# thanh-nt25/Whisper-context-biasing

Hardware: AMD Instinct MI355X
Metric: audio-seconds/sec (RTF) + biased-WER, whisper-small 30s clips, batch32 (higher is better)
Workload: dtype bf16

## Files before the change

whisper_context_biasing_amd/csrc/gemm_impl.h:

```cpp
#pragma once
#include <stdexcept>
#include <string>
#include "common.h"
#include "kernels.h"

#include <algorithm>
#include <cstdio>
#include <cstdlib>
#include <type_traits>

namespace wcb {

WCB_DEV void glds16(const void* gptr, void* lds_wave_base) {
  __builtin_amdgcn_global_load_lds(gptr, (__attribute__((address_space(3))) void*)lds_wave_base, 16, 0, 0);
}

WCB_DEV long a_row(const GemmArgs& g, int m) {
  return g.a_Mb ? (long)(m / g.a_Mb) * g.a_strideB + (long)(m % g.a_Mb) * g.lda : (long)m * g.lda;
}
WCB_DEV long c_row(const GemmArgs& g, int m) {
  return g.c_Mb ? (long)(m / g.c_Mb) * g.c_strideB + (long)(m % g.c_Mb) * g.ldc : (long)m * g.ldc;
}

enum : int { E_BIAS = 1, E_GELU = 2, E_RESID = 4, E_F32 = 8, E_ADDROW = 16, E_HEAD = 32, E_RUNTIME = 1 << 30 };
// ... 181 lines not shown
      for (int i = 0; i < FM; ++i)
#pragma unroll
        for (int j = 0; j < FN; ++j) acc[i][j] = mma16(a[i], b[j], acc[i][j]);
    }
    asm volatile("s_waitcnt vmcnt(0)" ::: "memory");
    __syncthreads();
  }

  constexpr int LDC = BN + 4;
  float* ct = reinterpret_cast<float*>(smem);
#pragma unroll
  for (int j = 0; j < FN; ++j) {
    const int col = wn * TN + j * 16 + (lane & 15);
    const int n = min(n0 + col, g.N - 1);
#pragma unroll
    for (int i = 0; i < FM; ++i)
#pragma unroll
      for (int e = 0; e < 4; ++e) {
        const int row = wm * TM + i * 16 + (lane >> 4) * 4 + e;
        const int m = min(m0 + row, g.M - 1);
        ct[row * LDC + col] = epi_pointwise<T, EPI>(g, m, n, acc[i][j][e]);
      }
  }
  __syncthreads();
  constexpr int C8 = BN / 8;
#pragma unroll 2
  for (int idx = tid; idx < BM * C8; idx += NT) {
    const int row = idx / C8, c8 = idx % C8;
    const int m = m0 + row;
    const int n = n0 + c8 * 8;
    if (m >= g.M || n >= g.N) continue;
    float v[8];
    const f32x4 lo = *reinterpret_cast<const f32x4*>(ct + row * LDC + c8 * 8);
    const f32x4 hi = *reinterpret_cast<const f32x4*>(ct + row * LDC + c8 * 8 + 4);
#pragma unroll
    for (int e = 0; e < 4; ++e) { v[e] = lo[e]; v[e + 4] = hi[e]; }
    epi_store8<T, EPI>(g, m, n, v);
  }
}

template <typename T, int BM, int BN, int WM, int WN, int NS, int EPI, bool LNF = false, int KT = 1, int BKB = 128,
          int PRIO = 0, bool WFM = false>
__global__ __launch_bounds__(WM * WN * 64) void gemm_ring_kernel(GemmArgs g) {
  constexpr int NW = WM * WN, NT = NW * 64;
  static_assert(BKB == 128 || BKB == 64, "LDS row: 128 or 64 bytes");
  constexpr int BK = BKB / 2, CE = 8;
  constexpr int CPR = BKB / 16, RPI = 64 / CPR, KS = BKB / 64;
  constexpr int TM = BM / WM, TN = BN / WN, FM = TM / 16, FN = TN / 16;
  constexpr int SUB = (BM + BN) * BKB, STAGE = SUB * KT;
  constexpr int IA = BM / RPI / NW, IB = BN / RPI / NW, GL = (IA + IB) * KT;
  static_assert(IA * NW * RPI == BM && IB * NW * RPI == BN, "tile rows must split over waves");
  auto swz = [](int r) { return BKB == 128 ? (r >> 1) & 7 : (r >> 2) & 3; };
  using Frag = typename DT<T>::frag;
  extern __shared__ __attribute__((aligned(16))) char smem[];

  const int tid = threadIdx.x, lane = tid & 63, wave = tid >> 6;
  const int wm = wave / WN, wn = wave % WN;
  const int tiles_n = (g.N + BN - 1) / BN;
  const int wg = xcd_remap(blockIdx.x, gridDim.x);
  int m0, n0;
  if (g.raster > 0) {
    const int tiles_m = (g.M + BM - 1) / BM, band = g.raster * tiles_n;
    const int fm = (wg / band) * g.raster, gm = min(tiles_m - fm, g.raster), r = wg % band;
    m0 = (fm + r % gm) * BM;
    n0 = (r / gm) * BN;
  } else {
    m0 = (wg / tiles_n) * BM;
    n0 = (wg % tiles_n) * BN;
  }

  const T* A = reinterpret_cast<const T*>(g.A);
  const T* W = reinterpret_cast<const T*>(g.W);
  const T* a_src[IA];
  const T* b_src[IB];
#pragma unroll
  for (int i = 0; i < IA; ++i) {
    const int r = (wave + i * NW) * RPI + lane / CPR;
    const int m = min(m0 + r, g.M - 1);
    a_src[i] = A + a_row(g, m) + ((lane % CPR) ^ swz(r)) * CE;
  }
  static_assert(!WFM || BKB == 128, "fragment-major W: 64-deep sub-tiles");
#pragma unroll
  for (int i = 0; i < IB; ++i) {
    const int r = (wave + i * NW) * RPI + lane / CPR;
    const long n = min(n0 + r, g.N - 1);
    const int c = (lane % CPR) ^ swz(r);
    if constexpr (WFM)
      b_src[i] = reinterpret_cast<const T*>(g.W_fm) + ((n / 16) * (g.K / 32) + c / 4) * 512 + (16 * (c % 4) + n % 16) * 8;
    else
      b_src[i] = W + n * g.ldw + c * CE;
  }
  constexpr int WKS = WFM ? 16 : 1;
  auto stage = [&](int st, int k0) {
#pragma unroll
    for (int t = 0; t < KT; ++t) {
      char* base = smem + st * STAGE + t * SUB;
#pragma unroll
      for (int i = 0; i < IA; ++i) glds16(a_src[i] + k0 + t * BK, base + (wave + i * NW) * 1024);
#pragma unroll
      for (int i = 0; i < IB; ++i) glds16(b_src[i] + (long)(k0 + t * BK) * WKS, base + BM * BKB + (wave + i * NW) * 1024);
    }
  };

  f32x4 acc[FM][FN];
#pragma unroll
  for (int i = 0; i < FM; ++i)
#pragma unroll
    for (int j = 0; j < FN; ++j) acc[i][j] = f32x4{0.f, 0.f, 0.f, 0.f};

  constexpr int LNF_OFF = NS * STAGE > BM * (BN + 4) * 4 ? NS * STAGE : BM * (BN + 4) * 4;
  float* lnraw = reinterpret_cast<float*>(smem + LNF_OFF);
  float* lnst = lnraw + BM * (kLnfMaxK / 32) * 2;
  const int nk = g.K / (BK * KT);
#pragma unroll
  for (int p = 0; p < NS - 1; ++p)
    if (p < nk) stage(p, p * BK * KT);
  if constexpr (LNF) {
    const int per_row = g.rst_nb * 8 / 16;
    const int chunks = BM * per_row;
    for (int q0 = wave * 64; q0 < chunks; q0 += NT) {
      const int q = min(q0 + lane, chunks - 1), r = q / per_row, j = q % per_row;
      const int m = min(m0 + r, g.M - 1);
      glds16(g.rst_in + ((long)m * g.rst_nb) * 2 + j * 4, reinterpret_cast<char*>(lnraw) + (long)q0 * 16);
    }
  }
  int st = 0;
  for (int kt = 0; kt < nk; ++kt) {
    const int ahead = min(nk - 1 - kt, NS - 2);
    if constexpr (NS >= 4) {
      static_assert(4 * GL <= 63, "vmcnt range");
      if (NS >= 6 && ahead >= 4) asm volatile("s_waitcnt vmcnt(%0)" :: "n"(4 * GL) : "memory");
      else if (NS >= 5 && ahead == 3) asm volatile("s_waitcnt vmcnt(%0)" :: "n"(3 * GL) : "memory");
      else if (ahead >= 2) asm volatile("s_waitcnt vmcnt(%0)" :: "n"(2 * GL) : "memory");
      else if (ahead == 1) asm volatile("s_waitcnt vmcnt(%0)" :: "n"(GL) : "memory");
      else asm volatile("s_waitcnt vmcnt(0)" ::: "memory");
    } else if constexpr (NS == 3) {
      if (ahead >= 1) asm volatile("s_waitcnt vmcnt(%0)" :: "n"(GL) : "memory");
      else asm volatile("s_waitcnt vmcnt(0)" ::: "memory");
    } else {
      asm volatile("s_waitcnt vmcnt(0)" ::: "memory");
    }
    __builtin_amdgcn_s_barrier();
    {
      const int nxt = kt + NS - 1;
      int sn = st + NS - 1;
      if (sn >= NS) sn -= NS;
      if (nxt < nk) stage(sn, nxt * BK * KT);
    }
#pragma unroll
    for (int kq = 0; kq < KS * KT; ++kq) {
      const char* base = smem + st * STAGE + (kq / KS) * SUB;
      const int ks = kq % KS;
      Frag a[FM], b[FN];
      const int c = ks * 4 + (lane >> 4);
#pragma unroll
      for (int i = 0; i < FM; ++i) {
        const int r = wm * TM + i * 16 + (lane & 15);
        a[i] = *reinterpret_cast<const Frag*>(base + r * BKB + ((c ^ swz(r)) << 4));
      }
#pragma unroll
      for (int j = 0; j < FN; ++j) {
        const int r = wn * TN + j * 16 + (lane & 15);
        b[j] = *reinterpret_cast<const Frag*>(base + BM * BKB + r * BKB + ((c ^ swz(r)) << 4));
      }
      if constexpr (PRIO == 1) __builtin_amdgcn_s_setprio(1);
#pragma unroll
      for (int i = 0; i < FM; ++i)
#pragma unroll
        for (int j = 0; j < FN; ++j) acc[i][j] = mma16(a[i], b[j], acc[i][j]);
      if constexpr (PRIO == 1) __builtin_amdgcn_s_setprio(0);
    }
    st = st + 1 == NS ? 0 : st + 1;
  }
  if constexpr (LNF) {
    __syncthreads();
    constexpr int LPR = NT / BM;
    static_assert(LPR >= 1 && (LPR & (LPR - 1)) == 0 && LPR <= 64, "lanes per row");
    const int r = tid / LPR, sub = tid % LPR;
    float a1 = 0.f, a2 = 0.f;
    for (int j = sub; j < g.rst_nb; j += LPR) {
      const float2 t = *reinterpret_cast<const float2*>(lnraw + ((long)r * g.rst_nb + j) * 2);
      a1 += t.x;
      a2 += t.y;
    }
#pragma unroll
    for (int o = 1; o < LPR; o <<= 1) { a1 += __shfl_xor(a1, o, 64); a2 += __shfl_xor(a2, o, 64); }
    if (sub == 0) {
      const float mean = a1 / g.K;
      lnst[2 * r] = mean;
      lnst[2 * r + 1] = rsqrtf(fmaxf(a2 / g.K - mean * mean, 0.f) + 1e-5f);
    }
  }
  __syncthreads();

  constexpr int LDC = BN + 4;
  constexpr int PASSES = (BM * LDC * 4 <= 160 * 1024) ? 1 : WM;
  constexpr int PR = BM / PASSES;
  float* ct = reinterpret_cast<float*>(smem);
#pragma unroll
  for (int ps = 0; ps < PASSES; ++ps) {
    if (PASSES == 1 || wm == ps) {
#pragma unroll
      for (int j = 0; j < FN; ++j) {
        const int col = wn * TN + j * 16 + (lane & 15);
#pragma unroll
        for (int i = 0; i < FM; ++i)
#pragma unroll
          for (int e = 0; e < 4; ++e) {
            const int row = wm * TM + i * 16 + (lane >> 4) * 4 + e;
            float v = acc[i][j][e];
            if constexpr (LNF) v = lnst[2 * row + 1] * (v - lnst[2 * row] * g.ln_u[min(n0 + col, g.N - 1)]);
            ct[(row - ps * PR) * LDC + col] = v;
          }
      }
    }
    __syncthreads();
    constexpr int C8 = BN / 8, RPIT = NT / C8;
    const int c8 = tid % C8;
    float b8[8] = {0.f, 0.f, 0.f, 0.f, 0.f, 0.f, 0.f, 0.f};
    if (has<EPI>(g, E_BIAS)) {
      const int nb = min(n0 + c8 * 8, g.N - 8);
      const f32x4 lo = *reinterpret_cast<const f32x4*>(g.bias + nb);
      const f32x4 hi = *reinterpret_cast<const f32x4*>(g.bias + nb + 4);
#pragma unroll
      for (int e = 0; e < 4; ++e) { b8[e] = lo[e]; b8[e + 4] = hi[e]; }
    }
    const int row0 = tid < RPIT * C8 ? tid / C8 : PR;
    constexpr int UNR = PR >= 2 * RPIT && EPI != E_RUNTIME ? 2 : 1;
#pragma unroll UNR
    for (int row = row0; row < PR; row += RPIT) {
      const int m = m0 + ps * PR + row;
      const int n = n0 + c8 * 8;
      const bool ok = m < g.M && n < g.N;
      float v[8];
      const f32x4 lo = *reinterpret_cast<const f32x4*>(ct + row * LDC + c8 * 8);
      const f32x4 hi = *reinterpret_cast<const f32x4*>(ct + row * LDC + c8 * 8 + 4);
#pragma unroll
      for (int e = 0; e < 4; ++e) { v[e] = lo[e]; v[e + 4] = hi[e]; }
#pragma unroll
      for (int e = 0; e < 8; ++e) {
        if (has<EPI>(g, E_BIAS)) v[e] += b8[e];
        if (has<EPI>(g, E_GELU)) v[e] = gelu_t<T>(v[e]);
        if (has<EPI>(g, E_ADDROW))
          v[e] += g.addrow[(long)(g.c_Mb ? min(m, g.M - 1) % g.c_Mb : min(m, g.M - 1)) * g.N + min(n + e, g.N - 1)];
      }
      if (ok) epi_store8<T, EPI>(g, m, n, v);
      if (EPI == E_RUNTIME && g.rst_out) {
        float a1 = 0.f, a2 = 0.f;
#pragma unroll
        for (int e = 0; e < 8; ++e) { a1 += v[e]; a2 = fmaf(v[e], v[e], a2); }
        a1 += __shfl_xor(a1, 1, 64); a2 += __shfl_xor(a2, 1, 64);
        a1 += __shfl_xor(a1, 2, 64); a2 += __shfl_xor(a2, 2, 64);
        if (ok && (c8 & 3) == 0) *reinterpret_cast<float2*>(g.rst_out + ((long)m * (g.N / 32) + n / 32) * 2) = float2{a1, a2};
      }
    }
    if (PASSES > 1) __syncthreads();
  }
}

template <typename T, int BM, int BN, int WM, int WN, int NS, int EPI, bool LNF = false, int KT = 1, int BKB = 128,
          int PRIO = 0, bool WFM = false>
static void launch_ring_e(const GemmArgs& g, hipStream_t s) {
  const int tiles = ((g.M + BM - 1) / BM) * ((g.N + BN - 1) / BN);
  constexpr int ring_bytes = NS * (BM + BN) * BKB * KT;
  constexpr int epi_full = BM * (BN + 4) * 4;
  constexpr int epi_bytes = epi_full <= 160 * 1024 ? epi_full : epi_full / WM;
  constexpr int base = ring_bytes > epi_bytes ? ring_bytes : epi_bytes;
  constexpr int lds = base + (LNF ? BM * (kLnfMaxK / 32) * 2 * 4 + 2 * BM * 4 : 0);
  static_assert(lds <= 160 * 1024, "LDS budget");
  static bool attr_set = false;
  if (!attr_set) {
    (void)hipFuncSetAttribute((const void*)gemm_ring_kernel<T, BM, BN, WM, WN, NS, EPI, LNF, KT, BKB, PRIO, WFM>,
                              hipFuncAttributeMaxDynamicSharedMemorySize, lds);
    attr_set = true;
  }
  WCB_LAUNCH((gemm_ring_kernel<T, BM, BN, WM, WN, NS, EPI, LNF, KT, BKB, PRIO, WFM>), dim3(tiles), dim3(WM * WN * 64), lds, s, g);
}

template <typename T, int BM, int BN, int NS, bool LNF, int KT = 1>
static void launch_ring_dec(const GemmArgs& g, hipStream_t s) {
  if (g.W_fm && g.K % 32 == 0) launch_ring_e<T, BM, BN, 2, 2, NS, E_RUNTIME, LNF, KT, 128, 0, true>(g, s);
  else launch_ring_e<T, BM, BN, 2, 2, NS, E_RUNTIME, LNF, KT>(g, s);
}

template <typename T, int BM, int BN, int WM, int WN, int NS, int BKB = 128, int PRIO = 1>
static void launch_ring(const GemmArgs& g, hipStream_t s) {
  const int bits = (g.bias ? E_BIAS : 0) | (g.act == 1 ? E_GELU : 0) | (g.resid ? E_RESID : 0) |
                   (g.out_f32 ? E_F32 : 0) | (g.addrow ? E_ADDROW : 0) | (g.mode == 1 ? E_HEAD : 0);
  switch (bits) {
    case E_BIAS: launch_ring_e<T, BM, BN, WM, WN, NS, E_BIAS, false, 1, BKB, PRIO>(g, s); break;
    case E_BIAS | E_GELU: launch_ring_e<T, BM, BN, WM, WN, NS, E_BIAS | E_GELU, false, 1, BKB, PRIO>(g, s); break;
    case E_BIAS | E_RESID | E_F32: launch_ring_e<T, BM, BN, WM, WN, NS, E_BIAS | E_RESID | E_F32, false, 1, BKB, PRIO>(g, s); break;
    case E_BIAS | E_GELU | E_F32 | E_ADDROW:
      launch_ring_e<T, BM, BN, WM, WN, NS, E_BIAS | E_GELU | E_F32 | E_ADDROW, false, 1, BKB, PRIO>(g, s); break;
    case E_BIAS | E_HEAD: launch_ring_e<T, BM, BN, WM, WN, NS, E_BIAS | E_HEAD, false, 1, BKB, PRIO>(g, s); break;
    default: launch_ring_e<T, BM, BN, WM, WN, NS, E_RUNTIME, false, 1, BKB, PRIO>(g, s); break;
  }
}

#ifdef WCB_GEMM_PROBE
__device__ unsigned long long* wcb_gemm_probe;
#define GPROBE(k)                                                                              \
  do {                                                                                         \
    if (threadIdx.x == 0) wcb_gemm_probe[blockIdx.x * 8 + (k)] = __builtin_amdgcn_s_memtime(); \
  } while (0)
#else
#define GPROBE(k) do {} while (0)
#endif
__device__ float wcb_pp_zeros[8192];
__device__ __attribute__((aligned(16))) char wcb_pp_scratch[64 * 16];

template <int N> WCB_DEV void vm_wait() { asm volatile("s_waitcnt vmcnt(%0)" :: "n"(N < 63 ? N : 63) : "memory"); }

template <typename T, int EPI, int BN = 256>
__global__ __launch_bounds__(512) void gemm_pp_kernel(GemmArgs g) {
  using Frag = typename DT<T>::frag;
  constexpr int BUF = 65536, WOFF = 32768;
  static_assert(BN == 256 || BN == 192, "tile width");
  constexpr int FW = BN / 64;
  constexpr int OPK = FW + 4;
  constexpr int S = 8 * FW + ((EPI & E_RESID) ? 8 * FW : 0);
  constexpr int BIAS_LDS = 2 * BUF;
  extern __shared__ __attribute__((aligned(16))) char smem[];
  const int tid = threadIdx.x, lane = tid & 63, wave = __builtin_amdgcn_readfirstlane(tid >> 6);
  const int wr = wave >> 2, wc = wave & 3;
  GPROBE(0);
  const int tiles_n = g.N / BN, tiles_m = (g.M + 255) >> 8, ntiles = tiles_m * tiles_n;
  const int nk = g.K >> 6;
  const int my = (ntiles - 1 - (int)blockIdx.x) / (int)gridDim.x + 1;
  const int total = my * nk;
  auto origin = [&](int it, int& m0, int& n0) {
    const int wg = xcd_remap((int)blockIdx.x + it * (int)gridDim.x, ntiles);
    if (g.raster > 0) {
      const int band = g.raster * tiles_n;
      const int fm = (wg / band) * g.raster, gm = min(tiles_m - fm, g.raster), r = wg % band;
      m0 = (fm + r % gm) * 256;
      n0 = (r / gm) * BN;
    } else {
      m0 = (wg / tiles_n) * 256;
      n0 = (wg % tiles_n) * BN;
    }
  };
  auto swzr = [](int r) { return (r >> 1) & 7; };
  const T* A = reinterpret_cast<const T*>(g.A);
  const T* W = reinterpret_cast<const T*>(g.W);
  const int i8 = 8 * wave + (lane >> 3), ch = lane & 7;
  const int m_last = (tiles_m - 1) * 256;
  int aoff[4], aoff_last[4], boff[4];
#pragma unroll
  for (int p = 0; p < 4; ++p) {
    const int ar = i8 < 32 ? 32 * p + i8 : 96 + 32 * p + i8;
    const int cs = (ch ^ swzr(ar)) << 3;
    aoff[p] = ar * (int)g.lda + cs;
    aoff_last[p] = (min(m_last + ar, g.M - 1) - m_last) * (int)g.lda + cs;
    boff[p] = (64 * min(p, FW - 1) + i8) * (int)g.ldw + ((ch ^ swzr(64 * p + i8)) << 3);
  }
  struct Cur { int it, kt, m0, n0; const T* a; const T* b; bool last; };
  auto set_tile = [&](Cur& c) {
    origin(c.it, c.m0, c.n0);
    c.a = A + (long)c.m0 * g.lda;
    c.b = W + (long)c.n0 * g.ldw;
    c.last = c.m0 == m_last;
  };
  auto advance = [&](Cur& c) {
    c.a += 64;
    c.b += 64;
    if (++c.kt == nk) {
      c.kt = 0;
      if (++c.it < my) set_tile(c);
    }
  };
  auto dma_a = [&](int p, const Cur& c, int gk) {
    glds16(c.a + (c.last ? aoff_last[p] : aoff[p]),
           smem + (gk & 1) * BUF + (wave < 4 ? 32 * p + 8 * wave : 96 + 32 * p + 8 * wave) * 128);
  };
  auto dma_b = [&](int t, const Cur& c, int gk) {
    glds16(c.b + boff[t], smem + (gk & 1) * BUF + WOFF + (64 * t + 8 * wave) * 128);
  };
  auto barrier = [] {
    __builtin_amdgcn_sched_barrier(0);
    __builtin_amdgcn_s_barrier();
    __builtin_amdgcn_sched_barrier(0);
  };

  f32x4 acc[8][FW];
#pragma unroll
  for (int i = 0; i < 8; ++i)
#pragma unroll
    for (int j = 0; j < FW; ++j) acc[i][j] = f32x4{0.f, 0.f, 0.f, 0.f};

  Cur cc;
  cc.it = 0; cc.kt = 0;
  set_tile(cc);
  Cur c1 = cc, c2 = cc;
  advance(c1);
  advance(c2);
  advance(c2);
  dma_b(0, cc, 0); dma_b(1, cc, 0); dma_a(0, cc, 0); dma_b(2, cc, 0);
  if constexpr (FW == 4) dma_b(3, cc, 0);
  dma_a(1, cc, 0); dma_a(2, cc, 0); dma_a(3, cc, 0);
  if (total > 1) {
    dma_b(0, c1, 1); dma_b(1, c1, 1); dma_a(0, c1, 1); dma_b(2, c1, 1);
    if constexpr (FW == 4) dma_b(3, c1, 1);
    dma_a(1, c1, 1);
  }
  GPROBE(1);
  if (total > 1) vm_wait<3 + FW + 2>();
  else vm_wait<3>();
  GPROBE(2);
  barrier();
  if (wr == 1) barrier();

  const int c0 = lane >> 4;
  const float* bias = g.bias ? g.bias : wcb_pp_zeros;
  const int sl = (lane >> 1) & 7;
  const int lo0 = (lane & 15) * 128 + ((c0 ^ sl) << 4), lo1 = (lane & 15) * 128 + (((4 + c0) ^ sl) << 4);
  const int wb0 = WOFF + 16 * FW * wc * 128 + lo0, wb1 = WOFF + 16 * FW * wc * 128 + lo1;
  const int ab0 = 128 * wr * 128 + lo0, ab1 = 128 * wr * 128 + lo1;
  auto ktile = [&](int gk, auto steady_tag) {
    constexpr bool ST = decltype(steady_tag)::value;
    const char* buf = smem + (gk & 1) * BUF;
    const bool n1 = ST || gk + 1 < total, n2 = ST || gk + 2 < total;
    const bool e0 = !ST && cc.kt == 0 && cc.it > 0, e1 = !ST && cc.kt == 1 && cc.it > 0;
    const bool plain = ST || (n2 && !e0 && !e1);
    Frag bw[FW][2];
#pragma unroll
    for (int p = 0; p < 4; ++p) {
      if (plain) {
        if (p < 3) vm_wait<OPK>();
        else vm_wait<6>();
      } else if (p == 0) {
        if (n1) { if (e0 || e1) vm_wait<OPK + S>(); else vm_wait<OPK>(); }
        else { if (e0 || e1) vm_wait<2 + S>(); else vm_wait<2>(); }
      } else if (p == 1) {
        if (n1) { if (e0) vm_wait<OPK + S>(); else vm_wait<OPK>(); }
        else { if (e0) vm_wait<1 + S>(); else vm_wait<1>(); }
      } else if (p == 2) {
        if (n1) { if (e0) vm_wait<OPK + S>(); else vm_wait<OPK>(); }
        else { if (e0) vm_wait<S>(); else vm_wait<0>(); }
      } else if (n1) {
        if (n2) { if (e0) vm_wait<6 + S>(); else vm_wait<6>(); }
        else { if (e0) vm_wait<3 + S>(); else vm_wait<3>(); }
      }
      if (p == 0) {
#pragma unroll
        for (int j = 0; j < FW; ++j) {
          bw[j][0] = *reinterpret_cast<const Frag*>(buf + wb0 + j * 16 * 128);
          bw[j][1] = *reinterpret_cast<const Frag*>(buf + wb1 + j * 16 * 128);
        }
      }
      if (!ST && p == 0 && cc.kt == 0 && wave == 0)
        glds16(bias + (BN == 256 ? cc.n0 + 4 * lane : min(cc.n0 + 4 * lane, g.N - 4)), smem + BIAS_LDS + (cc.it & 1) * 1024);
      Frag af[2][2];
#pragma unroll
      for (int i = 0; i < 2; ++i) {
        af[i][0] = *reinterpret_cast<const Frag*>(buf + ab0 + (32 * p + 16 * i) * 128);
        af[i][1] = *reinterpret_cast<const Frag*>(buf + ab1 + (32 * p + 16 * i) * 128);
      }
      if (p == 0 && n1) dma_a(2, c1, gk + 1);
      if (p == 1 && n1) dma_a(3, c1, gk + 1);
      if (p == 2 && n2) { dma_b(0, c2, gk + 2); dma_b(1, c2, gk + 2); dma_a(0, c2, gk + 2); }
      if (p == 3 && n2) {
        dma_b(2, c2, gk + 2);
        if constexpr (FW == 4) dma_b(3, c2, gk + 2);
        dma_a(1, c2, gk + 2);
      }
      barrier();
      asm volatile("s_waitcnt lgkmcnt(0)" ::: "memory");
      __builtin_amdgcn_s_setprio(1);
#pragma unroll
      for (int ks = 0; ks < 2; ++ks)
#pragma unroll
        for (int i = 0; i < 2; ++i)
#pragma unroll
          for (int j = 0; j < FW; ++j) acc[2 * p + i][j] = mma16(bw[j][ks], af[i][ks], acc[2 * p + i][j]);
      __builtin_amdgcn_s_setprio(0);
      barrier();
    }
  };
  for (int gk = 0; gk < total; ++gk) {
    ktile(gk, std::false_type{});
    if (gk == 0) GPROBE(3);
    if (gk == nk / 2) GPROBE(4);
    if (gk == 2 * nk - 1) GPROBE(7);
    if (cc.kt == nk - 1) {
      if (cc.it == 0) GPROBE(5);
      const int rb = cc.m0 + 128 * wr + (lane & 15);
      const int cb = cc.n0 + 16 * FW * wc + 4 * c0;
      f32x4 b4[FW];
#pragma unroll
      for (int j = 0; j < FW; ++j)
        b4[j] = *reinterpret_cast<const f32x4*>(smem + BIAS_LDS + (cc.it & 1) * 1024 + (16 * FW * wc + 4 * c0 + 16 * j) * 4);
#pragma unroll
      for (int mi = 0; mi < 8; ++mi) {
        const int m = rb + 16 * mi;
        const long off = (long)min(m, g.M - 1) * g.ldc + cb;
        f32x4 r4[FW];
        if constexpr ((EPI & E_RESID) != 0) {
#pragma unroll
          for (int j = 0; j < FW; ++j) r4[j] = *reinterpret_cast<const f32x4*>(g.resid + off + 16 * j);
        }
#pragma unroll
        for (int j = 0; j < FW; ++j) {
          f32x4 v = acc[mi][j] + b4[j];
          acc[mi][j] = f32x4{0.f, 0.f, 0.f, 0.f};
          if constexpr ((EPI & E_GELU) != 0) {
#pragma unroll
            for (int e = 0; e < 4; ++e) v[e] = gelu_t<T>(v[e]);
          }
          if constexpr ((EPI & E_RESID) != 0) v += r4[j];
          if constexpr ((EPI & E_F32) != 0) {
            float* dst = m < g.M ? reinterpret_cast<float*>(g.out) + off + 16 * j
                                 : reinterpret_cast<float*>(wcb_pp_scratch + lane * 16);
            *reinterpret_cast<f32x4*>(dst) = v;
          } else {
            typedef short s4 __attribute__((ext_vector_type(4)));
            s4 o;
#pragma unroll
            for (int e = 0; e < 4; ++e) o[e] = __builtin_bit_cast(short, DT<T>::fromf(v[e]));
            T* dst = m < g.M ? reinterpret_cast<T*>(g.out) + off + 16 * j : reinterpret_cast<T*>(wcb_pp_scratch + lane * 16);
            *reinterpret_cast<s4*>(dst) = o;
          }
        }
      }
      if (cc.it == 0) GPROBE(6);
    }
    cc = c1;
    c1 = c2;
    advance(c2);
  }
  if (wr == 0) barrier();
}

template <typename T, int EPI, int BN = 256>
static void launch_pp_e(const GemmArgs& g, hipStream_t s) {
  constexpr int kLds = 2 * 65536 + 2048;
  static bool attr_set = false;
  if (!attr_set) {
    (void)hipFuncSetAttribute((const void*)gemm_pp_kernel<T, EPI, BN>, hipFuncAttributeMaxDynamicSharedMemorySize, kLds);
    attr_set = true;
  }
  const int tiles = ((g.M + 255) / 256) * (g.N / BN);
  const dim3 grid((unsigned)(g.pp == 3 ? tiles : std::min(tiles, 256)));
  WCB_LAUNCH((gemm_pp_kernel<T, EPI, BN>), grid, dim3(512), kLds, s, g);
}

template <typename T>
static bool launch_pp(const GemmArgs& g, hipStream_t s) {
  if constexpr (sizeof(T) != 2) {
    return false;
  } else {
    const bool n256 = g.N % 256 == 0, n192 = g.N % 192 == 0;
    if ((!n256 && !n192) || g.N > 8192 || g.K % 64 != 0 || g.K < 128 || g.a_Mb || g.c_Mb || g.addrow || g.mode != 0 ||
        g.clamp != 0.f || g.rst_out || g.out16 || g.M < 256 || (g.resid && !g.out_f32) || (g.resid && g.act))
      return false;
    bool w192;
    if (g.pp == 2 || g.pp == 5) {
      w192 = g.pp == 5;
    } else {
      const long tm = (g.M + 255) / 256;
      const long r256 = n256 ? (tm * (g.N / 256) + 255) / 256 : 0, r192 = n192 ? (tm * (g.N / 192) + 255) / 256 : 0;
      w192 = !n256 || (n192 && r192 * 192 * 10 < r256 * 256 * 9);
      if (w192 && g.pp == 1) return false;
    }
    if ((w192 && !n192) || (!w192 && !n256)) return false;
    const int bits = (g.act == 1 ? E_GELU : 0) | (g.resid ? E_RESID : 0) | (g.out_f32 ? E_F32 : 0);
    if (w192) {
      switch (bits) {
        case 0: launch_pp_e<T, 0, 192>(g, s); return true;
        case E_GELU: launch_pp_e<T, E_GELU, 192>(g, s); return true;
        case E_F32: launch_pp_e<T, E_F32, 192>(g, s); return true;
        case E_RESID | E_F32: launch_pp_e<T, E_RESID | E_F32, 192>(g, s); return true;
        default: return false;
      }
    }
    switch (bits) {
      case 0: launch_pp_e<T, 0>(g, s); return true;
      case E_GELU: launch_pp_e<T, E_GELU>(g, s); return true;
      case E_F32: launch_pp_e<T, E_F32>(g, s); return true;
      case E_RESID | E_F32: launch_pp_e<T, E_RESID | E_F32>(g, s); return true;
      default: return false;
    }
  }
}

template <typename T, int MF, int NF, int NW, int KS, bool LN, bool SAMPLE = false>
__global__ __launch_bounds__(NW * 64) void gemm_skinny_kernel(GemmArgs g) {
  using Frag = typename DT<T>::frag;
  constexpr int NT = NW * 64, BNC = NF * 16;
  constexpr int SLAB = MF * 16 * (BNC + 1) * 4;
  constexpr int SL = (NW * SLAB <= 49152) ? NW : (NW / 2 * SLAB <= 49152) ? NW / 2 : (NW / 4 * SLAB <= 49152) ? NW / 4 : 1;
  __shared__ __attribute__((aligned(16))) float red[SL][MF * 16][BNC + 1];
  __shared__ float st_mean[MF * 16], st_rstd[MF * 16];
  const int tid = threadIdx.x, lane = tid & 63, wave = tid >> 6;
  const int mb = blockIdx.y * MF * 16;
  constexpr int NB = NW * KS * 2;
  constexpr int TPR = NB % 16 == 0 ? 16 : NB % 8 == 0 ? 8 : NB % 4 == 0 ? 4 : NB % 2 == 0 ? 2 : 1;
  constexpr int RPP = NT / TPR;
  constexpr int PASSES = (MF * 16 + RPP - 1) / RPP;
  float s1[PASSES], s2[PASSES];
  if constexpr (LN) {
#pragma unroll
    for (int ps = 0; ps < PASSES; ++ps) {
      const int m = min(mb + ps * RPP + tid / TPR, g.M - 1);
      s1[ps] = 0.f;
      s2[ps] = 0.f;
      float2 pv[NB / TPR];
#pragma unroll
      for (int j = 0; j < NB / TPR; ++j)
        pv[j] = *reinterpret_cast<const float2*>(g.st_in + ((long)m * NB + j * TPR + tid % TPR) * 2);
#pragma unroll
      for (int j = 0; j < NB / TPR; ++j) { s1[ps] += pv[j].x; s2[ps] += pv[j].y; }
    }
  }
  const int n0 = blockIdx.x * BNC;
  const int kb = wave * (KS * 32) + 8 * (lane >> 4);
  Frag b[NF][KS];
#pragma unroll
  for (int j = 0; j < NF; ++j) {
    const long n = min(n0 + j * 16 + (lane & 15), g.N - 1);
    const T* W = reinterpret_cast<const T*>(g.W) + n * g.ldw + kb;
#pragma unroll
    for (int ks = 0; ks < KS; ++ks) b[j][ks] = load_frag<T>(W + ks * 32);
  }
  constexpr int EP = (MF * 16 * BNC + NT - 1) / NT;
  float pf_bias[EP], pf_res[EP];
#pragma unroll
  for (int ep = 0; ep < EP; ++ep) {
    const int t = ep * NT + tid, row = mb + t / BNC, nn = n0 + t % BNC;
    const bool ok = t < MF * 16 * BNC && row < g.M && nn < g.N;
    pf_bias[ep] = (ok && g.bias) ? g.bias[nn] : 0.f;
    pf_res[ep] = (ok && g.resid && g.mode == 0) ? g.resid[c_row(g, row) + nn] : 0.f;
  }
  const int pos_v = g.mode == 2 ? *g.pos : 0;
  f32x4 acc[MF][NF];
#pragma unroll
  for (int i = 0; i < MF; ++i)
#pragma unroll
    for (int j = 0; j < NF; ++j) acc[i][j] = f32x4{0.f, 0.f, 0.f, 0.f};
  if constexpr (LN) {
    const float* X = reinterpret_cast<const float*>(g.A);
    float xv[MF][KS][8];
#pragma unroll
    for (int i = 0; i < MF; ++i) {
      const int m = min(mb + i * 16 + (lane & 15), g.M - 1);
      const float* xr = X + a_row(g, m) + kb;
#pragma unroll
      for (int ks = 0; ks < KS; ++ks) {
        const f32x4 x0 = *reinterpret_cast<const f32x4*>(xr + ks * 32);
        const f32x4 x1 = *reinterpret_cast<const f32x4*>(xr + ks * 32 + 4);
#pragma unroll
        for (int e = 0; e < 4; ++e) { xv[i][ks][e] = x0[e]; xv[i][ks][e + 4] = x1[e]; }
      }
    }
    float gw[KS][8], gb[KS][8];
#pragma unroll
    for (int ks = 0; ks < KS; ++ks) {
      const f32x4 w0 = *reinterpret_cast<const f32x4*>(g.ln_w + kb + ks * 32);
      const f32x4 w1 = *reinterpret_cast<const f32x4*>(g.ln_w + kb + ks * 32 + 4);
      const f32x4 b0 = *reinterpret_cast<const f32x4*>(g.ln_b + kb + ks * 32);
      const f32x4 b1 = *reinterpret_cast<const f32x4*>(g.ln_b + kb + ks * 32 + 4);
#pragma unroll
      for (int e = 0; e < 4; ++e) { gw[ks][e] = w0[e]; gw[ks][e + 4] = w1[e]; gb[ks][e] = b0[e]; gb[ks][e + 4] = b1[e]; }
    }
#pragma unroll
    for (int ps = 0; ps < PASSES; ++ps) {
      float a1 = s1[ps], a2 = s2[ps];
#pragma unroll
      for (int o = 1; o < TPR; o <<= 1) { a1 += __shfl_xor(a1, o, 64); a2 += __shfl_xor(a2, o, 64); }
      const int r = ps * RPP + tid / TPR;
      if (tid % TPR == 0 && r < MF * 16) {
        const float mean = a1 / g.K;
        st_mean[r] = mean;
        st_rstd[r] = rsqrtf(fmaxf(a2 / g.K - mean * mean, 0.f) + 1e-5f);
      }
    }
    __syncthreads();
#pragma unroll
    for (int i = 0; i < MF; ++i) {
      const float mean = st_mean[i * 16 + (lane & 15)], rstd = st_rstd[i * 16 + (lane & 15)];
#pragma unroll
      for (int ks = 0; ks < KS; ++ks) {
        Frag a;
#pragma unroll
        for (int e = 0; e < 8; ++e) {
          const float v = (xv[i][ks][e] - mean) * rstd * gw[ks][e] + gb[ks][e];
          if constexpr (sizeof(T) == 4) a[e] = v;
          else a[e] = __builtin_bit_cast(typename std::remove_reference<decltype(a[0])>::type, DT<T>::fromf(v));
        }
#pragma unroll
        for (int j = 0; j < NF; ++j) acc[i][j] = mma16(a, b[j][ks], acc[i][j]);
      }
    }
  } else {
    const T* A = reinterpret_cast<const T*>(g.A) + (g.a_grp_n ? (long)(n0 / g.a_grp_n) * g.a_grp_off : 0L);
#pragma unroll
    for (int i = 0; i < MF; ++i) {
      const int m = min(mb + i * 16 + (lane & 15), g.M - 1);
      const T* ap = A + a_row(g, m) + kb;
      Frag a[KS];
#pragma unroll
      for (int ks = 0; ks < KS; ++ks) a[ks] = load_frag<T>(ap + ks * 32);
#pragma unroll
      for (int ks = 0; ks < KS; ++ks)
#pragma unroll
        for (int j = 0; j < NF; ++j) acc[i][j] = mma16(a[ks], b[j][ks], acc[i][j]);
    }
  }
#pragma unroll
  for (int round = 0; round < NW / SL; ++round) {
    if (wave / SL == round) {
#pragma unroll
      for (int i = 0; i < MF; ++i)
#pragma unroll
        for (int j = 0; j < NF; ++j)
#pragma unroll
          for (int e = 0; e < 4; ++e) {
            float& r = red[wave % SL][i * 16 + (lane >> 4) * 4 + e][j * 16 + (lane & 15)];
            r = round == 0 ? acc[i][j][e] : r + acc[i][j][e];
          }
    }
    __syncthreads();
  }
  const bool mask_eos = g.sel_val && *g.sel_step < g.sel_min_new;
  const uint32_t* deny = !g.sel_val ? nullptr : (g.sel_deny0 && *g.sel_step == 0) ? g.sel_deny0 : g.sel_deny;
  [[maybe_unused]] int smp_step = 0;
  [[maybe_unused]] float smp_inv_t = 1.f;
  if constexpr (SAMPLE) { smp_step = *g.sel_step; smp_inv_t = *g.sel_inv_t; }
#pragma unroll
  for (int ep = 0; ep < EP; ++ep) {
    const int t = ep * NT + tid;
    const int lrow = t / BNC, col = t % BNC, row = mb + lrow;
    const int nn = n0 + col;
    const bool valid = t < MF * 16 * BNC && row < g.M && nn < g.N;
    float v = 0.f;
    if (valid) {
#pragma unroll
      for (int w = 0; w < SL; ++w) v += red[w][lrow][col];
      v += pf_bias[ep];
      if (g.act == 1) v = gelu_t<T>(v);
      if (g.addrow) v += g.addrow[(long)(g.c_Mb ? row % g.c_Mb : row) * g.N + nn];
      if (g.mode == 2 && nn >= g.n_split) {
        const int n2 = nn - g.n_split;
        const int hh = n2 >> 6, dd = n2 & 63;
        const int kv = hh / g.hs_H, h = hh % g.hs_H;
        const int rps = g.kv_rps > 1 ? g.kv_rps : 1;
        const long off = ((((long)kv * g.hs_B + row / rps) * g.hs_H + h) * g.kv_T + pos_v + row % rps) * 64 + dd;
        reinterpret_cast<T*>(g.kv_out)[off] = DT<T>::fromf(v);
      } else if (g.mode == 1) {
        v = epi_store1<T>(g, row, nn, v);
      } else {
        const long off = c_row(g, row) + nn;
        v += pf_res[ep];
        if (g.out_f32) reinterpret_cast<float*>(g.out)[off] = v;
        else reinterpret_cast<T*>(g.out)[off] = DT<T>::fromf(v);
      }
    }
    if (g.st_out) {
      float s1 = valid ? v : 0.f, s2 = valid ? v * v : 0.f;
#pragma unroll
      for (int o = 1; o < 16; o <<= 1) { s1 += __shfl_xor(s1, o, 64); s2 += __shfl_xor(s2, o, 64); }
      if (valid && (t & 15) == 0) {
        float* p = g.st_out + ((long)row * g.st_nb + blockIdx.x) * 2;
        p[0] = s1;
        p[1] = s2;
      }
    }
    if (g.sel_val) {
      float x = -INFINITY;
      int xi = 0x7fffffff;
      if (valid) {
        x = v;
        if (g.sel_lam != 0.f)
          x = bias_bonus(x, g.sel_lam, g.sel_rowbase[row] + (int)((g.sel_root_bits[nn >> 5] >> (nn & 31)) & 1u));
        if constexpr (SAMPLE) x = sample_perturb(x, smp_inv_t, sample_noise(g.sel_seeds[row], smp_step, nn));
        if (mask_eos && nn == g.sel_eos) x = -INFINITY;
        if (deny && deny_bit(deny, nn)) x = -INFINITY;
        xi = nn;
      }
#pragma unroll
      for (int o = 1; o < 64; o <<= 1) {
        const float ov = __shfl_xor(x, o, 64);
        const int oi = __shfl_xor(xi, o, 64);
        if (ov > x || (ov == x && oi < xi)) { x = ov; xi = oi; }
      }
      if (lane == 0 && row < g.M) {
        g.sel_val[(long)row * gridDim.x + blockIdx.x] = x;
        g.sel_idx[(long)row * gridDim.x + blockIdx.x] = xi;
      }
      if (g.sel_max) {
        float pm = valid ? v : -INFINITY, ps = valid ? 1.f : 0.f;
#pragma unroll
        for (int o = 1; o < 64; o <<= 1) {
          const float om = __shfl_xor(pm, o, 64), os = __shfl_xor(ps, o, 64);
          lse_merge(pm, ps, om, os);
        }
        if (lane == 0 && row < g.M) {
          g.sel_max[(long)row * gridDim.x + blockIdx.x] = pm;
          g.sel_sum[(long)row * gridDim.x + blockIdx.x] = ps;
        }
      }
    }
  }
}

template <typename T, int MF, int NW, int KPW, int AM, bool P, bool WFM = false, bool SAMPLE = false>
__global__ __launch_bounds__(NW * 64) void gemm_dec_kernel(GemmArgs g) {
  using Frag = typename DT<T>::frag;
  constexpr int NT = NW * 64, K = NW * KPW * 32, R = MF * 16;
  constexpr bool LN = AM == 1 || AM == 2;
  constexpr int EP = (R * 16 + NT - 1) / NT;
  __shared__ __attribute__((aligned(16))) float red[2][NW][R][17];
  __shared__ __attribute__((aligned(16))) float lnp[LN ? 2 * K : 4];
  __shared__ float2 rst[LN ? NW : 1][LN ? R : 1];
  const int tid = threadIdx.x, lane = tid & 63, wave = tid >> 6;
  const int mb = blockIdx.y * R;
  const int ntile = (g.N + 15) >> 4;
  const int kb = wave * (KPW * 32) + 8 * (lane >> 4);
  const int pos_v = g.mode == 2 ? *g.pos : 0;
  const bool mask_eos = g.sel_val && *g.sel_step < g.sel_min_new;

  auto load_w = [&](Frag (&w)[KPW], int ct) {
    if constexpr (WFM) {
      const T* W = reinterpret_cast<const T*>(g.W_fm) + (((long)ct * NW + wave) * KPW * 64 + lane) * 8;
#pragma unroll
      for (int ks = 0; ks < KPW; ++ks) w[ks] = __builtin_nontemporal_load(reinterpret_cast<const Frag*>(W + ks * 512));
    } else {
      const long n = min(ct * 16 + (lane & 15), g.N - 1);
      const T* W = reinterpret_cast<const T*>(g.W) + n * g.ldw + kb;
#pragma unroll
      for (int ks = 0; ks < KPW; ++ks) w[ks] = __builtin_nontemporal_load(reinterpret_cast<const Frag*>(W + ks * 32));
    }
  };
// ... 1266 lines not shown
```

Baseline: 20450.

## Prefetch residual rows into registers during last k-tile of pipelined GEMM

The residual-add epilogue of the persistent ping-pong GEMM now issues asynchronous residual loads during the final k-tile's last phase and streams the remaining groups while earlier groups are being stored. This hides residual fetch latency behind MMA work and stores. The tail handling is simplified by clamping the tile iterator so DMA is always issued, which removes the n1/n2 branching at the cost of redundant loads at the end. It also reworks the vmcnt wait accounting and adds register pressure for the residual buffers.

```diff
diff --git a/whisper_context_biasing_amd/csrc/gemm_impl.h b/whisper_context_biasing_amd/csrc/gemm_impl.h
--- a/whisper_context_biasing_amd/csrc/gemm_impl.h
+++ b/whisper_context_biasing_amd/csrc/gemm_impl.h
@@ -507,7 +507,7 @@
 __device__ unsigned long long* wcb_gemm_probe;
 #define GPROBE(k)                                                                              \
   do {                                                                                         \
-    if (threadIdx.x == 0) wcb_gemm_probe[blockIdx.x * 8 + (k)] = __builtin_amdgcn_s_memtime(); \
+    if (threadIdx.x == 0) wcb_gemm_probe[blockIdx.x * 16 + (k)] = __builtin_amdgcn_s_memtime(); \
   } while (0)
 #else
 #define GPROBE(k) do {} while (0)
@@ -524,7 +524,13 @@
   static_assert(BN == 256 || BN == 192, "tile width");
   constexpr int FW = BN / 64;
   constexpr int OPK = FW + 4;
-  constexpr int S = 8 * FW + ((EPI & E_RESID) ? 8 * FW : 0);
+  constexpr bool RS = (EPI & E_RESID) != 0;
+  constexpr int G0 = RS ? (FW == 3 ? 6 : 2) : 1, GB = RS ? 2 : 1;
+  constexpr int NB = 1 + (8 - G0) / GB;
+  constexpr int R = RS ? G0 * FW : 0;
+  constexpr int S = 8 * FW + (RS ? (8 - G0) * FW : 0);
+  static_assert(6 + S <= 63 && OPK + R <= 63, "a wait without a previous epilogue in it over the vmcnt range");
+  static_assert(OPK + R + S <= 63 || (RS && FW == 4), "only the 256-wide residual tile's e0 / e1 waits may over-wait");
   constexpr int BIAS_LDS = 2 * BUF;
   extern __shared__ __attribute__((aligned(16))) char smem[];
   const int tid = threadIdx.x, lane = tid & 63, wave = __builtin_amdgcn_readfirstlane(tid >> 6);
@@ -572,7 +578,8 @@
     c.b += 64;
     if (++c.kt == nk) {
       c.kt = 0;
-      if (++c.it < my) set_tile(c);
+      if (++c.it >= my) c.it = my - 1;
+      set_tile(c);
     }
   };
   auto dma_a = [&](int p, const Cur& c, int gk) {
@@ -604,14 +611,11 @@
   dma_b(0, cc, 0); dma_b(1, cc, 0); dma_a(0, cc, 0); dma_b(2, cc, 0);
   if constexpr (FW == 4) dma_b(3, cc, 0);
   dma_a(1, cc, 0); dma_a(2, cc, 0); dma_a(3, cc, 0);
-  if (total > 1) {
-    dma_b(0, c1, 1); dma_b(1, c1, 1); dma_a(0, c1, 1); dma_b(2, c1, 1);
-    if constexpr (FW == 4) dma_b(3, c1, 1);
-    dma_a(1, c1, 1);
-  }
+  dma_b(0, c1, 1); dma_b(1, c1, 1); dma_a(0, c1, 1); dma_b(2, c1, 1);
+  if constexpr (FW == 4) dma_b(3, c1, 1);
+  dma_a(1, c1, 1);
   GPROBE(1);
-  if (total > 1) vm_wait<3 + FW + 2>();
-  else vm_wait<3>();
+  vm_wait<3 + FW + 2>();
   GPROBE(2);
   barrier();
   if (wr == 1) barrier();
@@ -622,12 +626,23 @@
   const int lo0 = (lane & 15) * 128 + ((c0 ^ sl) << 4), lo1 = (lane & 15) * 128 + (((4 + c0) ^ sl) << 4);
   const int wb0 = WOFF + 16 * FW * wc * 128 + lo0, wb1 = WOFF + 16 * FW * wc * 128 + lo1;
   const int ab0 = 128 * wr * 128 + lo0, ab1 = 128 * wr * 128 + lo1;
-  auto ktile = [&](int gk, auto steady_tag) {
-    constexpr bool ST = decltype(steady_tag)::value;
+  f32x4 rr[G0][FW];
+#pragma unroll
+  for (int i = 0; i < G0; ++i)
+#pragma unroll
+    for (int j = 0; j < FW; ++j) rr[i][j] = f32x4{0.f, 0.f, 0.f, 0.f};
+  auto resid_load = [&](int grp, int slot) {
+    const int rb = cc.m0 + 128 * wr + (lane & 15);
+    const int cb = cc.n0 + 16 * FW * wc + 4 * c0;
+    const float* src = g.resid + (long)min(rb + 16 * grp, g.M - 1) * g.ldc + cb;
+#pragma unroll
+    for (int j = 0; j < FW; ++j)
+      asm volatile("global_load_dwordx4 %0, %1, off offset:%2" : "+v"(rr[slot][j]) : "v"(src), "n"(64 * j) : "memory");
+  };
+  auto ktile = [&](int gk) {
     const char* buf = smem + (gk & 1) * BUF;
-    const bool n1 = ST || gk + 1 < total, n2 = ST || gk + 2 < total;
-    const bool e0 = !ST && cc.kt == 0 && cc.it > 0, e1 = !ST && cc.kt == 1 && cc.it > 0;
-    const bool plain = ST || (n2 && !e0 && !e1);
+    const bool e0 = cc.kt == 0 && cc.it > 0, e1 = cc.kt == 1 && cc.it > 0;
+    const bool plain = !e0 && !e1;
     Frag bw[FW][2];
 #pragma unroll
     for (int p = 0; p < 4; ++p) {
@@ -635,17 +650,14 @@
         if (p < 3) vm_wait<OPK>();
         else vm_wait<6>();
       } else if (p == 0) {
-        if (n1) { if (e0 || e1) vm_wait<OPK + S>(); else vm_wait<OPK>(); }
-        else { if (e0 || e1) vm_wait<2 + S>(); else vm_wait<2>(); }
-      } else if (p == 1) {
-        if (n1) { if (e0) vm_wait<OPK + S>(); else vm_wait<OPK>(); }
-        else { if (e0) vm_wait<1 + S>(); else vm_wait<1>(); }
-      } else if (p == 2) {
-        if (n1) { if (e0) vm_wait<OPK + S>(); else vm_wait<OPK>(); }
-        else { if (e0) vm_wait<S>(); else vm_wait<0>(); }
-      } else if (n1) {
-        if (n2) { if (e0) vm_wait<6 + S>(); else vm_wait<6>(); }
-        else { if (e0) vm_wait<3 + S>(); else vm_wait<3>(); }
+        if (e0) vm_wait<OPK + R + S>();
+        else vm_wait<OPK + S>();
+      } else if (p < 3) {
+        if (e0) vm_wait<OPK + R + S>();
+        else vm_wait<OPK>();
+      } else {
+        if (e0) vm_wait<6 + S>();
+        else vm_wait<6>();
       }
       if (p == 0) {
 #pragma unroll
@@ -654,7 +666,7 @@
           bw[j][1] = *reinterpret_cast<const Frag*>(buf + wb1 + j * 16 * 128);
         }
       }
-      if (!ST && p == 0 && cc.kt == 0 && wave == 0)
+      if (p == 0 && cc.kt == 0 && wave == 0)
         glds16(bias + (BN == 256 ? cc.n0 + 4 * lane : min(cc.n0 + 4 * lane, g.N - 4)), smem + BIAS_LDS + (cc.it & 1) * 1024);
       Frag af[2][2];
 #pragma unroll
@@ -662,10 +674,16 @@
         af[i][0] = *reinterpret_cast<const Frag*>(buf + ab0 + (32 * p + 16 * i) * 128);
         af[i][1] = *reinterpret_cast<const Frag*>(buf + ab1 + (32 * p + 16 * i) * 128);
       }
-      if (p == 0 && n1) dma_a(2, c1, gk + 1);
-      if (p == 1 && n1) dma_a(3, c1, gk + 1);
-      if (p == 2 && n2) { dma_b(0, c2, gk + 2); dma_b(1, c2, gk + 2); dma_a(0, c2, gk + 2); }
-      if (p == 3 && n2) {
+      if (p == 0) dma_a(2, c1, gk + 1);
+      if (p == 1) dma_a(3, c1, gk + 1);
+      if (p == 2) { dma_b(0, c2, gk + 2); dma_b(1, c2, gk + 2); dma_a(0, c2, gk + 2); }
+      if (p == 3) {
+        if constexpr (RS) {
+          if (cc.kt == nk - 1) {
+#pragma unroll
+            for (int i = 0; i < G0; ++i) resid_load(i, i);
+          }
+        }
         dma_b(2, c2, gk + 2);
         if constexpr (FW == 4) dma_b(3, c2, gk + 2);
         dma_a(1, c2, gk + 2);
@@ -683,57 +701,86 @@
       barrier();
     }
   };
+  auto resid_landed = [&](int b) {
+    if (b == 0) vm_wait<FW - 1>();
+    else if (b == 1) vm_wait<G0 * FW>();
+    else vm_wait<GB * FW>();
+#pragma unroll
+    for (int i = 0; i < G0; ++i)
+#pragma unroll
+      for (int j = 0; j < FW; ++j)
+        if (b == 0 || i < GB) asm volatile("" : "+v"(rr[i][j]));
+  };
+  auto epilogue = [&] {
+    if (cc.it == 0) GPROBE(5);
+    const int rb = cc.m0 + 128 * wr + (lane & 15);
+    const int cb = cc.n0 + 16 * FW * wc + 4 * c0;
+    f32x4 b4[FW];
+#pragma unroll
+    for (int j = 0; j < FW; ++j)
+      b4[j] = *reinterpret_cast<const f32x4*>(smem + BIAS_LDS + (cc.it & 1) * 1024 + (16 * FW * wc + 4 * c0 + 16 * j) * 4);
+#pragma unroll
+    for (int b = 0; b < NB; ++b) {
+      const int g0 = b == 0 ? 0 : G0 + (b - 1) * GB, gn = b == 0 ? G0 : GB;
+      if constexpr (RS) resid_landed(b);
+#pragma unroll
+      for (int i = 0; i < G0; ++i)
+#pragma unroll
+        for (int j = 0; j < FW; ++j)
+          if (i < gn) {
+            f32x4 v = acc[g0 + i][j] + b4[j];
+            if constexpr ((EPI & E_GELU) != 0) {
+#pragma unroll
+              for (int e = 0; e < 4; ++e) v[e] = gelu_t<T>(v[e]);
+            }
+            if constexpr (RS) v += rr[i][j];
+            acc[g0 + i][j] = v;
+          }
+      if constexpr (RS) {
+        if (b + 1 < NB) {
+#pragma unroll
+          for (int i = 0; i < GB; ++i) resid_load(g0 + gn + i, i);
+        }
+      }
+#pragma unroll
+      for (int i = 0; i < G0; ++i)
+        if (i < gn) {
+          const int mi = g0 + i, m = rb + 16 * mi;
+          const long off = (long)min(m, g.M - 1) * g.ldc + cb;
+#pragma unroll
+          for (int j = 0; j < FW; ++j) {
+            const f32x4 v = acc[mi][j];
+            acc[mi][j] = f32x4{0.f, 0.f, 0.f, 0.f};
+            if constexpr ((EPI & E_F32) != 0) {
+              float* dst = m < g.M ? reinterpret_cast<float*>(g.out) + off + 16 * j
+                                   : reinterpret_cast<float*>(wcb_pp_scratch + lane * 16);
+              *reinterpret_cast<f32x4*>(dst) = v;
+            } else {
+              typedef short s4 __attribute__((ext_vector_type(4)));
+              s4 o;
+#pragma unroll
+              for (int e = 0; e < 4; ++e) o[e] = __builtin_bit_cast(short, DT<T>::fromf(v[e]));
+              T* dst = m < g.M ? reinterpret_cast<T*>(g.out) + off + 16 * j : reinterpret_cast<T*>(wcb_pp_scratch + lane * 16);
+              *reinterpret_cast<s4*>(dst) = o;
+            }
+          }
+        }
+    }
+    if (cc.it == 0) GPROBE(6);
+  };
   for (int gk = 0; gk < total; ++gk) {
-    ktile(gk, std::false_type{});
+    const bool lastk = cc.kt == nk - 1;
+    ktile(gk);
     if (gk == 0) GPROBE(3);
     if (gk == nk / 2) GPROBE(4);
+    if (gk == nk) GPROBE(8);
     if (gk == 2 * nk - 1) GPROBE(7);
-    if (cc.kt == nk - 1) {
-      if (cc.it == 0) GPROBE(5);
-      const int rb = cc.m0 + 128 * wr + (lane & 15);
-      const int cb = cc.n0 + 16 * FW * wc + 4 * c0;
-      f32x4 b4[FW];
-#pragma unroll
-      for (int j = 0; j < FW; ++j)
-        b4[j] = *reinterpret_cast<const f32x4*>(smem + BIAS_LDS + (cc.it & 1) * 1024 + (16 * FW * wc + 4 * c0 + 16 * j) * 4);
-#pragma unroll
-      for (int mi = 0; mi < 8; ++mi) {
-        const int m = rb + 16 * mi;
-        const long off = (long)min(m, g.M - 1) * g.ldc + cb;
-        f32x4 r4[FW];
-        if constexpr ((EPI & E_RESID) != 0) {
-#pragma unroll
-          for (int j = 0; j < FW; ++j) r4[j] = *reinterpret_cast<const f32x4*>(g.resid + off + 16 * j);
-        }
-#pragma unroll
-        for (int j = 0; j < FW; ++j) {
-          f32x4 v = acc[mi][j] + b4[j];
-          acc[mi][j] = f32x4{0.f, 0.f, 0.f, 0.f};
-          if constexpr ((EPI & E_GELU) != 0) {
-#pragma unroll
-            for (int e = 0; e < 4; ++e) v[e] = gelu_t<T>(v[e]);
-          }
-          if constexpr ((EPI & E_RESID) != 0) v += r4[j];
-          if constexpr ((EPI & E_F32) != 0) {
-            float* dst = m < g.M ? reinterpret_cast<float*>(g.out) + off + 16 * j
-                                 : reinterpret_cast<float*>(wcb_pp_scratch + lane * 16);
-            *reinterpret_cast<f32x4*>(dst) = v;
-          } else {
-            typedef short s4 __attribute__((ext_vector_type(4)));
-            s4 o;
-#pragma unroll
-            for (int e = 0; e < 4; ++e) o[e] = __builtin_bit_cast(short, DT<T>::fromf(v[e]));
-            T* dst = m < g.M ? reinterpret_cast<T*>(g.out) + off + 16 * j : reinterpret_cast<T*>(wcb_pp_scratch + lane * 16);
-            *reinterpret_cast<s4*>(dst) = o;
-          }
-        }
-      }
-      if (cc.it == 0) GPROBE(6);
-    }
+    if (lastk) epilogue();
     cc = c1;
     c1 = c2;
     advance(c2);
   }
+  vm_wait<0>();
   if (wr == 0) barrier();
 }
 
```

Result: slower. 20230 (-1.1%).
